# heiheishuang/MuDG

Hardware: AMD Instinct MI355X
Metric: DDIM denoise steps/sec, MDM1024 576x1024x16f (CFG: 2 UNet forwards + fused update per step, per clip) (higher is better)
Workload: dtype bf16; 1 GPU; MDM1024 latents (B=1,4,16,72,128) + c_concat 8ch, context (B,333,1024), 50-step uniform_trailing DDIM schedule, cfg 7.5, guidance_rescale 0.7, eta 1.0, v-prediction, dynamic rescale; clips_per_gpu=1, parallelism=clip-DP x1 (no in-step collective), launch=hipGraph replay of each UNet pass (cond+uncond batched)

## Files before the change

### mudg_amd/csrc/attention.hip

```cpp
#include "attn_shared.h"
#include <cstdlib>

namespace {

#if MUDG_PLANES == 1
template <bool TWO>
__global__ __launch_bounds__(256, 2) void attn_kernel(const MudgAttnDesc p, const int nqt, const int total) {
    __shared__ __attribute__((aligned(16))) h16 Ks[2 * ATILE];
    __shared__ __attribute__((aligned(16))) h16 Vs[2 * ATILE];

    const int tid = threadIdx.x, lane = tid & 63, wave = tid >> 6;
    const int l31 = lane & 31, hi = lane >> 5;

    const int w = xcd_work_item(total);
    const int pair = w / nqt, qt = w - pair * nqt;
    const int f = pair / p.heads, h = pair - f * p.heads;
    const h16* Qp = reinterpret_cast<const h16*>(p.Q) + (int64_t)f * p.Nq * p.ldq + h * 64;
    h16* Op = reinterpret_cast<h16*>(p.O) + (int64_t)f * p.Nq * p.ldo + h * 64;

    const int q = qt * QB + wave * 32 + l31;
    const bool qok = q < p.Nq;

    h16x8 qf[1][4];
    load_q_frags(qf[0], Qp, q, p.ldq, 0, qok, hi);

    const int lrow = tid >> 3, kc = tid & 7;
    u32x4 kr[1][2], vr[1][2];

    f32x16 o[2], res[TWO ? 2 : 1];
    const float c = p.q_prescaled ? 1.0f : p.scale * 1.4426950408889634f;
    float inv = 0.f;
#pragma unroll
    for (int set = 0; set < (TWO ? 2 : 1); ++set) {
        const KvSet kv = kv_set(p, f, h, set);
#pragma unroll
        for (int r = 0; r < 16; ++r) { o[0][r] = 0.f; o[1][r] = 0.f; }
        float m_run = -INFINITY, l_run = 0.f;

        const int nkt = (kv.Nk + KB - 1) / KB;
        load_kv_tile(kv, 0, lrow, kc, kr, vr);
        stage_padded(Ks, Vs, lrow, kc, kr, vr);
        __syncthreads();

        for (int kt = 0; kt < nkt; ++kt) {
            const int cur = kt & 1;
            const bool more = kt + 1 < nkt;
            if (more) load_kv_tile(kv, kt + 1, lrow, kc, kr, vr);
            FLASH_TILE(Ks + cur * ATILE, Vs + cur * ATILE, qf, kt, kv.Nk, c, m_run, l_run, o, l31, hi);
            if (more) stage_padded(Ks + (cur ^ 1) * ATILE, Vs + (cur ^ 1) * ATILE, lrow, kc, kr, vr);
            __syncthreads();
        }
        inv = finish_set<TWO>(p, set, f, h, q, qok, hi, c, m_run, l_run, o, res);
    }
    if (qok) store_o16(o, inv, Op + (int64_t)q * p.ldo, hi, p.accumulate);
}

constexpr int XK_TILES = 3;
template <bool TWO>
__global__ __launch_bounds__(256, 2) void xattn_kernel(const MudgAttnDesc p, const int nqt, const int xq, const int nqc, const int total) {
    extern __shared__ __attribute__((aligned(16))) h16 xlds[];
    h16* Ks = xlds;
    h16* Vs = xlds + XK_TILES * ATILE;
    const int tid = threadIdx.x, lane = tid & 63, wave = tid >> 6;
    const int l31 = lane & 31, hi = lane >> 5;
    const int w = xcd_work_item(total);
    const int pair = w / nqc, qc = w - pair * nqc;
    const int f = pair / p.heads, h = pair - f * p.heads;
    const h16* Qp = reinterpret_cast<const h16*>(p.Q) + (int64_t)f * p.Nq * p.ldq + h * 64;
    h16* Op = reinterpret_cast<h16*>(p.O) + (int64_t)f * p.Nq * p.ldo + h * 64;
    const int nt0 = (p.Nk + KB - 1) / KB;

    {
        const int lrow = tid >> 3, kc = tid & 7;
#pragma unroll
        for (int set = 0; set < (TWO ? 2 : 1); ++set) {
            const KvSet kv = kv_set(p, f, h, set);
            const int nkt = (kv.Nk + KB - 1) / KB;
            for (int kt = 0; kt < nkt; ++kt) {
                const int ti = set == 0 ? kt : nt0 + kt;
                u32x4 kr[1][2], vr[1][2];
                load_kv_tile(kv, kt, lrow, kc, kr, vr);
                stage_padded(Ks + ti * ATILE, Vs + ti * ATILE, lrow, kc, kr, vr);
            }
        }
    }
    __syncthreads();

    const float c = p.q_prescaled ? 1.0f : p.scale * 1.4426950408889634f;
    for (int qi = 0; qi < xq; ++qi) {
        const int qt = qc * xq + qi;
        if (qt >= nqt) break;
        const int q = qt * QB + wave * 32 + l31;
        const bool qok = q < p.Nq;
        h16x8 qf[1][4];
        load_q_frags(qf[0], Qp, q, p.ldq, 0, qok, hi);
        f32x16 o[2], res[TWO ? 2 : 1];
        float inv = 0.f;
#pragma unroll
        for (int set = 0; set < (TWO ? 2 : 1); ++set) {
            const int Nk = set == 0 ? p.Nk : p.Nk2;
#pragma unroll
            for (int r = 0; r < 16; ++r) { o[0][r] = 0.f; o[1][r] = 0.f; }
            float m_run = -INFINITY, l_run = 0.f;
            const int nkt = (Nk + KB - 1) / KB;
            for (int kt = 0; kt < nkt; ++kt) {
                const int ti = set == 0 ? kt : nt0 + kt;
                FLASH_TILE(Ks + ti * ATILE, Vs + ti * ATILE, qf, kt, Nk, c, m_run, l_run, o, l31, hi);
            }
            inv = finish_set<TWO>(p, set, f, h, q, qok, hi, c, m_run, l_run, o, res);
        }
        if (qok) store_o16(o, inv, Op + (int64_t)q * p.ldo, hi, p.accumulate);
    }
}

__global__ __launch_bounds__(256, 2) void attn64q_kernel(const MudgAttnDesc p, const int nqt, const int total) {
    __shared__ __attribute__((aligned(16))) h16 Ks[2 * ATILE];
    __shared__ __attribute__((aligned(16))) h16 Vs[2 * ATILE];

    const int tid = threadIdx.x, lane = tid & 63, wave = tid >> 6;
    const int l31 = lane & 31, hi = lane >> 5;
    const int w = xcd_work_item(total);
    const int pair = w / nqt, qt = w - pair * nqt;
    const int f = pair / p.heads, h = pair - f * p.heads;
    const KvSet kv = kv_set(p, f, h, 0);

    const h16* Qp = reinterpret_cast<const h16*>(p.Q) + (int64_t)f * p.Nq * p.ldq + h * 64;
    h16* Op = reinterpret_cast<h16*>(p.O) + (int64_t)f * p.Nq * p.ldo + h * 64;

    int qrow[2];
    bool qok[2];
    h16x8 qf[2][4];
#pragma unroll
    for (int qb = 0; qb < 2; ++qb) {
        qrow[qb] = qt * 256 + wave * 64 + qb * 32 + l31;
        qok[qb] = qrow[qb] < p.Nq;
        load_q_frags(qf[qb], Qp, qrow[qb], p.ldq, 0, qok[qb], hi);
    }

    const int lrow = tid >> 3, kc = tid & 7;
    u32x4 kr[1][2], vr[1][2];
    const int vlo = (kc >> 1) * 16 + ((kc & 1) ? 4 : 0), vhi = (kc >> 1) * 16 + ((kc & 1) ? 12 : 8);
    auto stage = [&](int buf) {
#pragma unroll
        for (int i = 0; i < 2; ++i) {
            st16(&Ks[buf * ATILE + (lrow + 32 * i) * ALD + kc * 8], kr[0][i]);
// ... 461 lines not shown
        __builtin_amdgcn_wave_barrier();
#pragma unroll
        for (int s = 0; s < 2; ++s) {
            const int r = lr + 8 * s;
            st16(qs + r * 128 + ((lj ^ (r & 7)) << 4), qn[s]);
            st16(ks + r * 128 + ((lj ^ (r & 7)) << 4), kn[s]);
            const int z = tattn_fz(r >> 2);
            u32x2 lo = {vn[s][0], vn[s][1]}, hi = {vn[s][2], vn[s][3]};
            *reinterpret_cast<u32x2*>(vs + r * 128 + (((2 * lj) ^ z) << 3)) = lo;
            *reinterpret_cast<u32x2*>(vs + r * 128 + (((2 * lj + 1) ^ z) << 3)) = hi;
        }
        __builtin_amdgcn_wave_barrier();
        if (it + 1 < TATTN_ITEMS) fetch(w0 + it + 1);

        float ov[16];
        tattn_item_mfma(qs, ks, vs, c, g, T, scale, ov);
        if (c < T) {
            h16* dst = O + (pix + (int64_t)c * HW) * ldo + h * 64 + g * 8;
#pragma unroll
            for (int half = 0; half < 2; ++half) {
                h16x8 t;
#pragma unroll
                for (int e = 0; e < 8; ++e) t[e] = (h16)ov[half * 8 + e];
                st16(dst + half * 32, as_u32x4(t));
            }
        }
    }
}

constexpr int TSA_KT = 64;
constexpr int TSA_ROWS = 128, TSA_COLS = 192;
constexpr int TSA_STAGE = (TSA_ROWS + TSA_COLS) * TSA_KT * 2;
constexpr int TSA_LDS = 2 * TSA_STAGE;
static_assert(TSA_LDS >= 4 * 2 * 3 * 2048, "the dead stages must hold 4 waves x 2 items x 3 tiles (q, k, v) x 2 KB");

__global__ __launch_bounds__(256, 2) void tsattn_fused_kernel(const h16* __restrict__ X, const h16* __restrict__ W, h16* __restrict__ O,
                                                               const int HW, const int heads, const int C, const int64_t ldx,
                                                               const int64_t ldw, const int64_t ldo, const float scale, const int total) {
    extern __shared__ __attribute__((aligned(16))) char tsa_smem[];
    const int tid = threadIdx.x, lane = tid & 63, wave = tid >> 6;
    const int c = lane & 15, g = lane >> 4;
    const int item = xcd_work_item(total);
    const int tile = item / heads, h = item - tile * heads;
    const int tpc = HW >> 3;
    const int b = tile / tpc, px0 = (tile - b * tpc) << 3;
    const int64_t row0 = (int64_t)b * 16 * HW + px0;

    const int lrow = tid >> 3, lch = tid & 7;
    const h16* src[10];
#pragma unroll
    for (int i = 0; i < 4; ++i) {
        const int r = lrow + 32 * i;
        src[i] = X + (row0 + (int64_t)(r & 15) * HW + (r >> 4)) * ldx + lch * 8;
    }
#pragma unroll
    for (int i = 0; i < 6; ++i) src[4 + i] = W + (int64_t)(h * TSA_COLS + lrow + 32 * i) * ldw + lch * 8;
    const int soff = lrow * 128 + ((lch ^ (lrow & 7)) << 4);

    u32x4 nx[10];
    auto fetch = [&](int kt) {
#pragma unroll
        for (int i = 0; i < 10; ++i) nx[i] = ld16(src[i] + kt * TSA_KT);
    };
    auto stage = [&](char* st) {
#pragma unroll
        for (int i = 0; i < 10; ++i) st16(st + soff + 4096 * i, nx[i]);
    };

    f32x4 acc[2][12];
#pragma unroll
    for (int pi = 0; pi < 2; ++pi)
#pragma unroll
        for (int nb = 0; nb < 12; ++nb) acc[pi][nb] = f32x4{0.f, 0.f, 0.f, 0.f};

    const int nk = C / TSA_KT;
    fetch(0);
    stage(tsa_smem);
    __syncthreads();
    for (int kt = 0; kt < nk; ++kt) {
        const char* cur = tsa_smem + (kt & 1) * TSA_STAGE;
        if (kt + 1 < nk) fetch(kt + 1);
#pragma unroll
        for (int s = 0; s < 2; ++s) {
            const int foff = c * 128 + (((g + 4 * s) ^ (c & 7)) << 4);
            const h16x8 xf0 = as_h16x8(ld16(cur + (32 * wave) * 128 + foff));
            const h16x8 xf1 = as_h16x8(ld16(cur + (32 * wave + 16) * 128 + foff));
#pragma unroll
            for (int nb = 0; nb < 12; ++nb) {
                const h16x8 wf = as_h16x8(ld16(cur + (TSA_ROWS + 16 * nb) * 128 + foff));
                acc[0][nb] = MFMA_16x16x32(wf, xf0, acc[0][nb]);
                acc[1][nb] = MFMA_16x16x32(wf, xf1, acc[1][nb]);
            }
        }
        if (kt + 1 < nk) stage(tsa_smem + ((kt + 1) & 1) * TSA_STAGE);
        __syncthreads();
    }

    char* mine = tsa_smem + wave * (2 * 3 * 2048);
#pragma unroll
    for (int pi = 0; pi < 2; ++pi) {
        char* qs = mine + pi * (3 * 2048);
#pragma unroll
        for (int nb = 0; nb < 12; ++nb) {
            Pack8 t;
#pragma unroll
            for (int i = 0; i < 4; ++i) t.h[i] = (h16)acc[pi][nb][i];
            const int u = 4 * (nb & 3) + g;
            const int off = (nb >> 2) == 2 ? c * 128 + ((u ^ tattn_fz(c >> 2)) << 3)
                                           : c * 128 + (((u >> 1) ^ (c & 7)) << 4) + ((u & 1) << 3);
            *reinterpret_cast<u32x2*>(qs + (nb >> 2) * 2048 + off) = t.u;
        }
    }
    __builtin_amdgcn_wave_barrier();
#pragma unroll
    for (int pi = 0; pi < 2; ++pi) {
        const char* qs = mine + pi * (3 * 2048);
        float ov[16];
        tattn_item_mfma(qs, qs + 2048, qs + 4096, c, g, 16, scale, ov);
        h16* dst = O + (row0 + (int64_t)c * HW + (2 * wave + pi)) * ldo + h * 64 + g * 8;
#pragma unroll
        for (int half = 0; half < 2; ++half) {
            h16x8 t;
#pragma unroll
            for (int e = 0; e < 8; ++e) t[e] = (h16)ov[half * 8 + e];
            st16(dst + half * 32, as_u32x4(t));
        }
    }
}
#endif

#if MUDG_PLANES > 1
template <bool TWO>
__global__ __launch_bounds__(256, PLANES == 2 ? 2 : 1) void attn_split_kernel(const MudgAttnDesc p, const int nqt, const int total) {
    extern __shared__ __attribute__((aligned(16))) char smem_raw[];
    h16* Ks = reinterpret_cast<h16*>(smem_raw);
    h16* Vs = Ks + 2 * PLANES * ATILE;

    const int tid = threadIdx.x, lane = tid & 63, wave = tid >> 6;
    const int l31 = lane & 31, hi = lane >> 5;
    const int w = xcd_work_item(total);
    const int pair = w / nqt, qt = w - pair * nqt;
    const int f = pair / p.heads, h = pair - f * p.heads;
    const int psq = p.ldq / PLANES, pso = p.ldo / PLANES;

    const h16* Qp = reinterpret_cast<const h16*>(p.Q) + (int64_t)f * p.Nq * p.ldq + h * 64;
    h16* Op = reinterpret_cast<h16*>(p.O) + (int64_t)f * p.Nq * p.ldo + h * 64;

    const int q = qt * QB + wave * 32 + l31;
    const bool qok = q < p.Nq;
    h16x8 qf[PLANES][4];
#pragma unroll
    for (int pl = 0; pl < PLANES; ++pl) load_q_frags(qf[pl], Qp, q, p.ldq, pl * psq, qok, hi);

    const int lrow = tid >> 3, kc = tid & 7;
    u32x4 kr[PLANES][2], vr[PLANES][2];

    f32x16 o[2], res[TWO ? 2 : 1];
    const float c = p.q_prescaled ? 1.0f : p.scale * 1.4426950408889634f;
#pragma unroll
    for (int set = 0; set < (TWO ? 2 : 1); ++set) {
// ... 426 lines not shown
#endif
        if (dma_ok) {
#if MUDG_PLANES == 2
            if (const int rc = mudg_lds_opt_in<&attn_split_dma_kernel<true>>(SPLIT_DMA_SMEM, "mudg_attention")) return rc;
            if (const int rc = mudg_lds_opt_in<&attn_split_dma_kernel<false>>(SPLIT_DMA_SMEM, "mudg_attention")) return rc;
            if (d.q_prescaled) hipLaunchKernelGGL(attn_split_dma_kernel<true>, dim3((unsigned)total), dim3(256), SPLIT_DMA_SMEM, s, d, nqt, (int)total);
            else hipLaunchKernelGGL(attn_split_dma_kernel<false>, dim3((unsigned)total), dim3(256), SPLIT_DMA_SMEM, s, d, nqt, (int)total);
#endif
        }
        else if (d.K2) hipLaunchKernelGGL(attn_split_kernel<true>, dim3((unsigned)total), dim3(256), smem, s, d, nqt, (int)total);
        else hipLaunchKernelGGL(attn_split_kernel<false>, dim3((unsigned)total), dim3(256), smem, s, d, nqt, (int)total);
    }
#else
    MUDG_REQUIRE(!d.Q8 || wide, "mudg_attention: the MX-fp8 score path serves the long self-attention kernel only (Nq >= 512, Nk >= 256)");
    if (wide) {
        const int nqt2 = (d.Nq + 255) / 256;
        const int64_t total2 = (int64_t)nqt2 * d.F * d.heads;
        static int dma = -1, lean = -1;
        if (dma < 0) dma = mudg_variant("ATTN_DMA", 1);
        if (lean < 0) lean = mudg_variant("ATTN_LEAN", 1);
        const bool dma_ok = dma && d.Nk % 64 == 0 && (int64_t)d.Nk * d.ldk * 2 < (1ll << 31) && (int64_t)64 * d.ldvt * 2 + (int64_t)d.Nk * 2 < (1ll << 31);
        if (d.Q8) {
            MUDG_REQUIRE(dma_ok && d.q_prescaled && d.K8 && d.Qs && d.Ks && !d.accumulate, "mudg_attention: the MX-fp8 score path needs "
                         "q_prescaled, Nk %% 64 == 0 and all four of Q8 / K8 / Qs / Ks");
            MUDG_REQUIRE((d.ldq8 & 15) == 0 && (d.ldk8 & 15) == 0 && aligned16(d.Q8) && aligned16(d.K8) && d.ldq8 >= d.heads * 64 &&
                         d.ldk8 >= d.heads * 64 && d.ldqs >= d.heads * 2 && d.ldks >= d.heads * 2 && (int64_t)d.Nk * d.ldk8 < (1ll << 31),
                         "mudg_attention: fp8 strides");
            hipLaunchKernelGGL((attn64d_kernel<true, true>), dim3((unsigned)total2), dim3(256), 0, s, d, nqt2, (int)total2);
        }
        else if (dma_ok && d.q_prescaled && lean) hipLaunchKernelGGL((attn64d_kernel<true, false>), dim3((unsigned)total2), dim3(256), 0, s, d, nqt2, (int)total2);
        else if (dma_ok) hipLaunchKernelGGL((attn64d_kernel<false, false>), dim3((unsigned)total2), dim3(256), 0, s, d, nqt2, (int)total2);
        else hipLaunchKernelGGL(attn64q_kernel, dim3((unsigned)total2), dim3(256), 0, s, d, nqt2, (int)total2);
    } else {
        static int xv = -1;
        if (xv < 0) xv = mudg_variant("ATTN_X", 1);
        int xq = (int)(total / 1024);
        xq = xq > 8 ? 8 : xq;
        if (xv && xq >= 2 && d.Nk <= 2 * KB && (!d.K2 || d.Nk2 <= KB)) {
            constexpr int smem = 2 * XK_TILES * ATILE * (int)sizeof(h16);
            if (const int rc = mudg_lds_opt_in<&xattn_kernel<false>>(smem, "mudg_attention")) return rc;
            if (const int rc = mudg_lds_opt_in<&xattn_kernel<true>>(smem, "mudg_attention")) return rc;
            const int nqc = (nqt + xq - 1) / xq;
            const int64_t totx = (int64_t)nqc * d.F * d.heads;
            if (d.K2) hipLaunchKernelGGL(xattn_kernel<true>, dim3((unsigned)totx), dim3(256), smem, s, d, nqt, xq, nqc, (int)totx);
            else hipLaunchKernelGGL(xattn_kernel<false>, dim3((unsigned)totx), dim3(256), smem, s, d, nqt, xq, nqc, (int)totx);
        }
        else if (d.K2) hipLaunchKernelGGL(attn_kernel<true>, dim3((unsigned)total), dim3(256), 0, s, d, nqt, (int)total);
        else hipLaunchKernelGGL(attn_kernel<false>, dim3((unsigned)total), dim3(256), 0, s, d, nqt, (int)total);
    }
#endif
    const int rc = mudg_check_launch("mudg_attention");
    const double bh = (double)d.F * d.heads;
    mudg_prof_end(slot, s, 4.0 * bh * d.Nq * (double)(d.Nk + (d.K2 ? d.Nk2 : 0)) * 64.0,
                  bh * (2.0 * d.Nq + 2.0 * d.Nk / d.kv_div + (d.K2 ? 2.0 * d.Nk2 / d.kv_div2 : 0.0)) * 64.0 * 2.0);
    return rc;
}

#if MUDG_PLANES == 1
namespace {
__global__ __launch_bounds__(256) void quantize_mxfp8_kernel(const h16* __restrict__ X, int ldx, int64_t rows, int nblk,
                                                              unsigned char* __restrict__ Y, int ldy, unsigned char* __restrict__ S, int lds) {
    const int64_t i = (int64_t)blockIdx.x * 256 + threadIdx.x;
    if (i >= rows * nblk) return;
    const int64_t r = i / nblk;
    const int b = (int)(i - r * nblk);
    const h16* src = X + r * ldx + b * 32;
    float v[32];
    float amax = 0.f;
#pragma unroll
    for (int q = 0; q < 4; ++q) {
        const h16x8 t = as_h16x8(ld16(src + q * 8));
#pragma unroll
        for (int e = 0; e < 8; ++e) { v[q * 8 + e] = (float)t[e]; amax = fmaxf(amax, fabsf(v[q * 8 + e])); }
    }
    const int E = mx_block_exponent(amax);
    const float inv = __uint_as_float((unsigned)(127 - E) << 23);
    u32x4 lo, hi4;
#pragma unroll
// ... 55 lines not shown
#endif
    if (T <= 16) launch(tattn_split_kernel<16>, 4);
    else launch(tattn_split_kernel<32>, 4);
#else
    if (T <= 16 && use_mfma) launch(tattn_mfma_kernel, 4 * TATTN_ITEMS);
    else if (T <= 16) launch(tattn_kernel<16>, 4 * TATTN_ITEMS);
    else launch(tattn_kernel<32>, 4 * TATTN_ITEMS);
#endif
    const int rc = mudg_check_launch("mudg_temporal_attention");
    mudg_prof_end(slot, s, 4.0 * total * (double)T * T * 64.0, (double)total * T * 64.0 * 2.0 * 4.0);
    return rc;
}

extern "C" int mudg_temporal_self_attention_ok(int T, int HW, int heads, int C, int64_t ldx, int64_t ldw, int64_t ldo) {
#if MUDG_PLANES == 1
    return T == 16 && HW > 0 && HW % 8 == 0 && heads > 0 && C == heads * 64 && ldx % 8 == 0 && ldw % 8 == 0 && ldo % 8 == 0 && ldx >= C &&
           ldw >= C && ldo >= C;
#else
    (void)T; (void)HW; (void)heads; (void)C; (void)ldx; (void)ldw; (void)ldo;
    return 0;
#endif
}

extern "C" int mudg_temporal_self_attention(const void* X, const void* Wh, void* O, int B, int T, int HW, int heads, int C, int64_t ldx,
                                            int64_t ldw, int64_t ldo, float scale, void* stream) {
#if MUDG_PLANES == 1
    MUDG_REQUIRE(X && Wh && O, "mudg_temporal_self_attention: null pointer");
    MUDG_REQUIRE(B > 0, "mudg_temporal_self_attention: empty problem");
    MUDG_REQUIRE(aligned16(X) && aligned16(Wh) && aligned16(O), "mudg_temporal_self_attention: alignment");
    if (!mudg_temporal_self_attention_ok(T, HW, heads, C, ldx, ldw, ldo))
        MUDG_FAIL(MUDG_EUNSUPPORTED, "mudg_temporal_self_attention: T=%d HW=%d heads=%d C=%d outside the fused kernel (T = 16, HW %% 8 == 0, "
                  "C = 64 heads, dense 16-byte rows): project with mudg_gemm and call mudg_temporal_attention", T, HW, heads, C);
    const int64_t total = (int64_t)B * (HW / 8) * heads;
    MUDG_REQUIRE(total < (1ll << 31), "mudg_temporal_self_attention: grid too large");
    const int rc0 = mudg_lds_opt_in<tsattn_fused_kernel>(TSA_LDS, "mudg_temporal_self_attention");
    if (rc0 != MUDG_OK) return rc0;
    hipStream_t s = reinterpret_cast<hipStream_t>(stream);
    const int slot = mudg_prof_begin(MUDG_FAM_GEMM, s);
    hipLaunchKernelGGL(tsattn_fused_kernel, dim3((unsigned)total), dim3(256), TSA_LDS, s, (const h16*)X, (const h16*)Wh, (h16*)O, HW, heads, C,
                       ldx, ldw, ldo, scale, (int)total);
    const int rc = mudg_check_launch("mudg_temporal_self_attention");
    const double M = (double)B * T * HW;
    mudg_prof_end(slot, s, 2.0 * M * 3.0 * C * C + 4.0 * (double)B * HW * heads * T * T * 64.0, (2.0 * M * C + 3.0 * C * C) * 2.0);
    return rc;
#else
    (void)X; (void)Wh; (void)O; (void)B; (void)T; (void)HW; (void)heads; (void)C; (void)ldx; (void)ldw; (void)ldo; (void)scale; (void)stream;
    MUDG_FAIL(MUDG_EUNSUPPORTED, "mudg_temporal_self_attention: the fused kernel belongs to the 16-bit operand builds");
#endif
}
```

### mudg_amd/csrc/attn_shared.h

```cpp
#pragma once
#include "common.h"
#include <type_traits>

constexpr int QB = 128;
constexpr int KB = 64;
constexpr int ALD = 72;
constexpr int ATILE = 64 * ALD;

struct KvSet {
    const h16* Kp;
    const h16* Vp;
    int Nk, ldk, ldvt;
    int psk, psv;
};
__device__ __forceinline__ KvSet kv_set(const MudgAttnDesc& p, int f, int h, int set) {
    KvSet kv;
    if (set == 0) {
        kv.Kp = reinterpret_cast<const h16*>(p.K) + (int64_t)(f / p.kv_div) * p.Nk * p.ldk + h * 64;
        kv.Vp = reinterpret_cast<const h16*>(p.Vt) + (int64_t)(f / p.kv_div) * p.svt + (int64_t)(h * 64) * p.ldvt;
        kv.Nk = p.Nk; kv.ldk = p.ldk; kv.ldvt = p.ldvt;
    } else {
        kv.Kp = reinterpret_cast<const h16*>(p.K2) + (int64_t)(f / p.kv_div2) * p.Nk2 * p.ldk2 + h * 64;
        kv.Vp = reinterpret_cast<const h16*>(p.Vt2) + (int64_t)(f / p.kv_div2) * p.svt2 + (int64_t)(h * 64) * p.ldvt2;
        kv.Nk = p.Nk2; kv.ldk = p.ldk2; kv.ldvt = p.ldvt2;
// ... 11 lines not shown
__device__ __forceinline__ void load_kv_tile(const KvSet& kv, int kt, int lrow, int kc, u32x4 (&kr)[PLANES][2], u32x4 (&vr)[PLANES][2]) {
    const int j0 = kt * KB;
#pragma unroll
    for (int pl = 0; pl < PLANES; ++pl)
#pragma unroll
        for (int i = 0; i < 2; ++i) {
            const int row = lrow + 32 * i;
            const int j = j0 + row;
            kr[pl][i] = (j < kv.Nk) ? ld16(kv.Kp + (int64_t)j * kv.ldk + pl * kv.psk + kc * 8) : zero16();
            const int jc = j0 + kc * 8;
            u32x4 v = zero16();
            if (jc < kv.Nk) {
                v = ld16(kv.Vp + (int64_t)row * kv.ldvt + pl * kv.psv + jc);
                if (jc + 8 > kv.Nk) {
                    h16x8 hv = as_h16x8(v);
#pragma unroll
                    for (int e = 0; e < 8; ++e) if (jc + e >= kv.Nk) hv[e] = (h16)0.f;
                    v = as_u32x4(hv);
                }
            }
            vr[pl][i] = v;
        }
}
__device__ __forceinline__ void stage_padded(h16* Kt, h16* Vt, int lrow, int kc, const u32x4 (&kr)[PLANES][2], const u32x4 (&vr)[PLANES][2]) {
#pragma unroll
    for (int pl = 0; pl < PLANES; ++pl)
#pragma unroll
        for (int i = 0; i < 2; ++i) {
            st16(&Kt[pl * ATILE + (lrow + 32 * i) * ALD + kc * 8], kr[pl][i]);
            st16(&Vt[pl * ATILE + (lrow + 32 * i) * ALD + kc * 8], vr[pl][i]);
        }
}

__device__ __forceinline__ void mask_ragged(f32x16 (&s)[2], int kt, int Nk, int hi) {
    if (kt * KB + KB > Nk) {
#pragma unroll
        for (int sub = 0; sub < 2; ++sub)
#pragma unroll
            for (int r = 0; r < 16; ++r) {
                const int j = kt * KB + sub * 32 + (r & 3) + 8 * (r >> 2) + 4 * hi;
                if (j >= Nk) s[sub][r] = -INFINITY;
            }
    }
}

__device__ __forceinline__ float row_max32(const f32x16 (&s)[2]) {
    float mx = s[0][0];
#pragma unroll
    for (int r = 1; r < 16; ++r) mx = fmaxf(mx, s[0][r]);
#pragma unroll
    for (int r = 0; r < 16; ++r) mx = fmaxf(mx, s[1][r]);
    return fmaxf(mx, __shfl_xor(mx, 32, 64));
}

__device__ __forceinline__ void put_p(h16x8 (&pk)[PLANES][2][2], int sub, int r, float e) {
    h16 piece[PLANES];
    split_operand(e, piece);
#pragma unroll
    for (int pl = 0; pl < PLANES; ++pl) pk[pl][sub][r >> 3][r & 7] = piece[pl];
}

__device__ __forceinline__ void softmax_step_classic(const f32x16 (&s)[2], float c, float& m_run, float& l_run, f32x16 (&o)[2],
                                                     h16x8 (&pk)[PLANES][2][2]) {
    const float mx = row_max32(s);
    const bool grew = !__all(mx <= m_run);
    const float m_new = grew ? fmaxf(m_run, mx) : m_run;
    const float alpha = grew ? __builtin_amdgcn_exp2f((m_run - m_new) * c) : 1.0f;
    const float mc = m_new * c;
    m_run = m_new;
    float ps = 0.f;
#pragma unroll
    for (int sub = 0; sub < 2; ++sub)
#pragma unroll
        for (int r = 0; r < 16; ++r) {
            const float e = __builtin_amdgcn_exp2f(fmaf(s[sub][r], c, -mc));
            ps += e;
            put_p(pk, sub, r, e);
        }
    l_run = l_run * alpha + ps;
    if (grew) {
#pragma unroll
        for (int r = 0; r < 16; ++r) { o[0][r] *= alpha; o[1][r] *= alpha; }
    }
}

#ifdef MUDG_OPERAND_FP16
constexpr float LEAN_LIMIT = 32768.f;
#else
constexpr float LEAN_LIMIT = 1099511627776.f;
#endif
__device__ __forceinline__ bool softmax_step_lean(const f32x16 (&s)[2], float& l_run, h16x8 (&pk)[PLANES][2][2]) {
    float ps = 0.f;
#pragma unroll
    for (int sub = 0; sub < 2; ++sub)
#pragma unroll
        for (int r = 0; r < 16; ++r) {
            const float e = __builtin_amdgcn_exp2f(s[sub][r]);
            ps += e;
            put_p(pk, sub, r, e);
        }
    l_run += ps;
    return !(ps <= LEAN_LIMIT);
}
template <bool LEAN, class KeyLoop>
__device__ __forceinline__ void lean_or_classic(const bool& overflow, KeyLoop key_loop) {
    if constexpr (LEAN) {
        key_loop(std::true_type{});
        if (__syncthreads_or(overflow ? 1 : 0)) key_loop(std::false_type{});
    } else {
        key_loop(std::false_type{});
    }
}

#define FLASH_TILE(Kt, Vt, qf, kt, Nk, c, m_run, l_run, o, l31, hi) do {                                                  \
    const h16* const ft_K = (Kt); const h16* const ft_V = (Vt); const int ft_kt = (kt), ft_Nk = (Nk);                     \
    f32x16 ft_s[2];                                                                                                       \
    _Pragma("unroll") for (int sub = 0; sub < 2; ++sub) {                                                                 \
        _Pragma("unroll") for (int r = 0; r < 16; ++r) ft_s[sub][r] = 0.f;                                                \
        _Pragma("unroll") for (int sg = 0; sg < NSEG; ++sg) {                                                             \
            const h16* kp = ft_K + seg_xp(sg) * ATILE + (sub * 32 + (l31)) * ALD + (hi) * 8;                              \
            _Pragma("unroll") for (int ks = 0; ks < 4; ++ks) {                                                            \
                const h16x8 kf = *reinterpret_cast<const h16x8*>(kp + ks * 16);                                           \
                ft_s[sub] = MFMA_32x32x16(kf, (qf)[seg_wp(sg)][ks], ft_s[sub]);                                           \
            }                                                                                                             \
        }                                                                                                                 \
    }                                                                                                                     \
    mask_ragged(ft_s, ft_kt, ft_Nk, (hi));                                                                                \
    h16x8 ft_pk[PLANES][2][2];                                                                                            \
    softmax_step_classic(ft_s, (c), (m_run), (l_run), (o), ft_pk);                                                        \
    _Pragma("unroll") for (int dt = 0; dt < 2; ++dt)                                                                      \
        _Pragma("unroll") for (int sg = 0; sg < NSEG; ++sg) {                                                             \
            const h16* vp = ft_V + seg_xp(sg) * ATILE + (dt * 32 + (l31)) * ALD + 4 * (hi);                               \
            _Pragma("unroll") for (int sub = 0; sub < 2; ++sub)                                                           \
                _Pragma("unroll") for (int jj = 0; jj < 2; ++jj) {                                                        \
                    const int kk = sub * 32 + jj * 16;                                                                    \
                    const h16x4 lo = *reinterpret_cast<const h16x4*>(vp + kk);                                            \
                    const h16x4 up = *reinterpret_cast<const h16x4*>(vp + kk + 8);                                        \
                    h16x8 vf;                                                                                             \
                    _Pragma("unroll") for (int e = 0; e < 4; ++e) { vf[e] = lo[e]; vf[4 + e] = up[e]; }                   \
                    (o)[dt] = MFMA_32x32x16(vf, ft_pk[seg_wp(sg)][sub][jj], (o)[dt]);                                     \
                }                                                                                                         \
        }                                                                                                                 \
} while (0)

__device__ __forceinline__ void store_lse(const MudgAttnDesc& p, int f, int h, int q, bool qok, int hi, float c, float m_run, float l_tot) {
    if (p.Lse && qok && hi == 0) p.Lse[((int64_t)f * p.Nq + q) * p.heads + h] = m_run * c + __log2f(l_tot);
}
__device__ __forceinline__ void store_o16(const f32x16 (&o)[2], float inv, h16* orow, int hi, int accumulate) {
#pragma unroll
    for (int dt = 0; dt < 2; ++dt)
#pragma unroll
        for (int g = 0; g < 4; ++g) {
            h16* dst = orow + dt * 32 + 8 * g + 4 * hi;
            float v[4];
#pragma unroll
            for (int j = 0; j < 4; ++j) v[j] = o[dt][4 * g + j] * inv;
            if (accumulate) {
                Pack8 old; old.u = *reinterpret_cast<const u32x2*>(dst);
#pragma unroll
                for (int j = 0; j < 4; ++j) v[j] += (float)old.h[j];
            }
            Pack8 nw;
#pragma unroll
            for (int j = 0; j < 4; ++j) nw.h[j] = (h16)v[j];
            *reinterpret_cast<u32x2*>(dst) = nw.u;
        }
}
template <bool TWO>
__device__ __forceinline__ float finish_set(const MudgAttnDesc& p, int set, int f, int h, int q, bool qok, int hi, float c,
                                            float m_run, float l_run, f32x16 (&o)[2], f32x16 (&res)[TWO ? 2 : 1]) {
    const float l_tot = l_run + __shfl_xor(l_run, 32, 64);
    float inv = 1.f / l_tot;
    if (!TWO) store_lse(p, f, h, q, qok, hi, c, m_run, l_tot);
    if (TWO) {
        if (set == 0) {
#pragma unroll
            for (int r = 0; r < 16; ++r) { res[0][r] = o[0][r] * inv; res[1][r] = o[1][r] * inv; }
        } else {
#pragma unroll
            for (int r = 0; r < 16; ++r) { o[0][r] = fmaf(o[0][r], inv, res[0][r]); o[1][r] = fmaf(o[1][r], inv, res[1][r]); }
            inv = 1.f;
        }
    }
    return inv;
}
__device__ __forceinline__ void finish_block16(const MudgAttnDesc& p, int f, int h, int q, bool qok, int hi, float c,
                                               float m_run, float l_run, const f32x16 (&o)[2], h16* Op) {
    const float l_tot = l_run + __shfl_xor(l_run, 32, 64);
    const float inv = 1.f / l_tot;
    store_lse(p, f, h, q, qok, hi, c, m_run, l_tot);
    if (qok) store_o16(o, inv, Op + (int64_t)q * p.ldo, hi, p.accumulate);
}

__device__ __forceinline__ __amdgpu_buffer_rsrc_t attn_rsrc(const h16* base) {
    return __builtin_amdgcn_make_buffer_rsrc(const_cast<h16*>(base), 0, (int)0x80000000u, 0x00020000);
}
typedef __attribute__((address_space(3))) void* attn_lptr_t;
__device__ __forceinline__ int swap_mid4(int row) {
    const int i16 = row & 15;
    return (row & ~15) | (i16 & 3) | ((i16 & 8) >> 1) | ((i16 & 4) << 1);
// ... 11 lines not shown
```

Baseline: 8.790 steps/s.

## Make fused temporal self-attention persistent with async LDS buffer loads

Converts the fused temporal self-attention kernel from one workgroup per item into a persistent grid of two workgroups per CU, each walking a contiguous range of items. Operand tiles are now fetched with buffer loads that write straight to LDS, interleaved with the MFMA loop, and the next item's first stage is prefetched while the current item's attention epilogue runs. This is meant to remove register staging, launch tail effects and the exposed load latency at item boundaries. It adds hand-placed vmcnt waits and barriers with fixed counts, and an out-of-bounds offset trick for the final prefetch, which are fragile if the tile shape changes.

```diff
diff --git a/mudg_amd/csrc/attention.hip b/mudg_amd/csrc/attention.hip
--- a/mudg_amd/csrc/attention.hip
+++ b/mudg_amd/csrc/attention.hip
@@ -638,100 +638,145 @@
 constexpr int TSA_ROWS = 128, TSA_COLS = 192;
 constexpr int TSA_STAGE = (TSA_ROWS + TSA_COLS) * TSA_KT * 2;
 constexpr int TSA_LDS = 2 * TSA_STAGE;
-static_assert(TSA_LDS >= 4 * 2 * 3 * 2048, "the dead stages must hold 4 waves x 2 items x 3 tiles (q, k, v) x 2 KB");
+constexpr int TSA_XP = TSA_ROWS / 8 / 4, TSA_WP = TSA_COLS / 8 / 4;
+constexpr int TSA_STORES = 2 * 2;
+constexpr unsigned TSA_OOB = 0x80000000u;
+static_assert(TSA_STAGE >= 4 * 3 * 2048, "a dead stage must hold 4 waves x 3 tiles (q, k, v) x 2 KB");
+static_assert(TSA_XP + TSA_WP == 10 && TSA_STORES == 4, "TSA_WAIT_ITEM below is TSA_STORES");
+#define TSA_WAIT_STAGE() asm volatile("s_waitcnt vmcnt(0)" ::: "memory")
+#define TSA_WAIT_ITEM() asm volatile("s_waitcnt vmcnt(4)" ::: "memory")
+#define TSA_BARRIER()                          \
+    do {                                       \
+        __builtin_amdgcn_sched_barrier(0);     \
+        __builtin_amdgcn_s_barrier();          \
+        __builtin_amdgcn_sched_barrier(0);     \
+    } while (0)
 
 __global__ __launch_bounds__(256, 2) void tsattn_fused_kernel(const h16* __restrict__ X, const h16* __restrict__ W, h16* __restrict__ O,
                                                                const int HW, const int heads, const int C, const int64_t ldx,
                                                                const int64_t ldw, const int64_t ldo, const float scale, const int total) {
     extern __shared__ __attribute__((aligned(16))) char tsa_smem[];
-    const int tid = threadIdx.x, lane = tid & 63, wave = tid >> 6;
+    const int tid = threadIdx.x, lane = tid & 63;
+    const int wave = __builtin_amdgcn_readfirstlane(tid >> 6);
     const int c = lane & 15, g = lane >> 4;
-    const int item = xcd_work_item(total);
-    const int tile = item / heads, h = item - tile * heads;
-    const int tpc = HW >> 3;
-    const int b = tile / tpc, px0 = (tile - b * tpc) << 3;
-    const int64_t row0 = (int64_t)b * 16 * HW + px0;
-
-    const int lrow = tid >> 3, lch = tid & 7;
-    const h16* src[10];
-#pragma unroll
-    for (int i = 0; i < 4; ++i) {
-        const int r = lrow + 32 * i;
-        src[i] = X + (row0 + (int64_t)(r & 15) * HW + (r >> 4)) * ldx + lch * 8;
-    }
-#pragma unroll
-    for (int i = 0; i < 6; ++i) src[4 + i] = W + (int64_t)(h * TSA_COLS + lrow + 32 * i) * ldw + lch * 8;
-    const int soff = lrow * 128 + ((lch ^ (lrow & 7)) << 4);
-
-    u32x4 nx[10];
-    auto fetch = [&](int kt) {
-#pragma unroll
-        for (int i = 0; i < 10; ++i) nx[i] = ld16(src[i] + kt * TSA_KT);
-    };
-    auto stage = [&](char* st) {
-#pragma unroll
-        for (int i = 0; i < 10; ++i) st16(st + soff + 4096 * i, nx[i]);
+    const int nwg = (int)gridDim.x, wg = xcd_work_item(nwg);
+    const int per = total / nwg, rem = total % nwg;
+    const int i0 = wg * per + (wg < rem ? wg : rem), i1 = i0 + per + (wg < rem ? 1 : 0);
+    if (i0 == i1) return;
+    const int nk = C / TSA_KT;
+
+    auto next_item = [&](int& h, int& px0, int& b) {
+        if (++h == heads) {
+            h = 0;
+            px0 += 8;
+            if (px0 == HW) { px0 = 0; ++b; }
+        }
+    };
+    int h, px0, b;
+    {
+        const int tile = i0 / heads, tpc = HW >> 3;
+        h = i0 - tile * heads;
+        b = tile / tpc;
+        px0 = (tile - b * tpc) << 3;
+    }
+    int nit = i0, nkt = 0, nh = h, npx0 = px0, nb = b;
+
+    const int lrow = lane >> 3, lch = (lane & 7) ^ lrow;
+    const int ldx2 = (int)ldx * 2, ldw2 = (int)ldw * 2;
+    const unsigned vx = (unsigned)lrow * (unsigned)HW * (unsigned)ldx2 + (unsigned)lch * 16u;
+    const unsigned vw = (unsigned)lrow * (unsigned)ldw2 + (unsigned)lch * 16u;
+    __amdgpu_buffer_rsrc_t rX, rW;
+    unsigned ux, uw;
+    int ko;
+    auto aim = [&]() {
+        const bool live = nit < i1;
+        rX = attn_rsrc(X + ((int64_t)nb * 16 * HW + npx0) * ldx);
+        rW = attn_rsrc(W + (int64_t)nh * TSA_COLS * ldw);
+        ux = live ? vx : TSA_OOB, uw = live ? vw : TSA_OOB;
+        ko = nkt * (TSA_KT * 2);
+    };
+    auto piece = [&](char* buf, const int j) {
+        if (j < TSA_XP)
+            __builtin_amdgcn_raw_ptr_buffer_load_lds(rX, (attn_lptr_t)(buf + (TSA_XP * wave + j) * 1024), 16, (int)ux,
+                                                     ((j & 1) * 8 * HW + 2 * wave + (j >> 1)) * ldx2 + ko, 0, 0);
+        else
+            __builtin_amdgcn_raw_ptr_buffer_load_lds(rW, (attn_lptr_t)(buf + (TSA_ROWS / 8 + TSA_WP * wave + (j - TSA_XP)) * 1024), 16, (int)uw,
+                                                     (8 * TSA_WP * wave + 8 * (j - TSA_XP)) * ldw2 + ko, 0, 0);
+    };
+    auto advance = [&]() {
+        if (++nkt == nk) { nkt = 0; ++nit; next_item(nh, npx0, nb); }
+    };
+    auto issue = [&](char* buf) {
+        aim();
+#pragma unroll
+        for (int j = 0; j < TSA_XP + TSA_WP; ++j) piece(buf, j);
+        advance();
     };
 
     f32x4 acc[2][12];
 #pragma unroll
     for (int pi = 0; pi < 2; ++pi)
 #pragma unroll
-        for (int nb = 0; nb < 12; ++nb) acc[pi][nb] = f32x4{0.f, 0.f, 0.f, 0.f};
-
-    const int nk = C / TSA_KT;
-    fetch(0);
-    stage(tsa_smem);
-    __syncthreads();
-    for (int kt = 0; kt < nk; ++kt) {
-        const char* cur = tsa_smem + (kt & 1) * TSA_STAGE;
-        if (kt + 1 < nk) fetch(kt + 1);
-#pragma unroll
-        for (int s = 0; s < 2; ++s) {
-            const int foff = c * 128 + (((g + 4 * s) ^ (c & 7)) << 4);
-            const h16x8 xf0 = as_h16x8(ld16(cur + (32 * wave) * 128 + foff));
-            const h16x8 xf1 = as_h16x8(ld16(cur + (32 * wave + 16) * 128 + foff));
-#pragma unroll
-            for (int nb = 0; nb < 12; ++nb) {
-                const h16x8 wf = as_h16x8(ld16(cur + (TSA_ROWS + 16 * nb) * 128 + foff));
-                acc[0][nb] = MFMA_16x16x32(wf, xf0, acc[0][nb]);
-                acc[1][nb] = MFMA_16x16x32(wf, xf1, acc[1][nb]);
-            }
-        }
-        if (kt + 1 < nk) stage(tsa_smem + ((kt + 1) & 1) * TSA_STAGE);
-        __syncthreads();
-    }
-
-    char* mine = tsa_smem + wave * (2 * 3 * 2048);
-#pragma unroll
-    for (int pi = 0; pi < 2; ++pi) {
-        char* qs = mine + pi * (3 * 2048);
-#pragma unroll
-        for (int nb = 0; nb < 12; ++nb) {
-            Pack8 t;
-#pragma unroll
-            for (int i = 0; i < 4; ++i) t.h[i] = (h16)acc[pi][nb][i];
-            const int u = 4 * (nb & 3) + g;
-            const int off = (nb >> 2) == 2 ? c * 128 + ((u ^ tattn_fz(c >> 2)) << 3)
-                                           : c * 128 + (((u >> 1) ^ (c & 7)) << 4) + ((u & 1) << 3);
-            *reinterpret_cast<u32x2*>(qs + (nb >> 2) * 2048 + off) = t.u;
-        }
-    }
-    __builtin_amdgcn_wave_barrier();
-#pragma unroll
-    for (int pi = 0; pi < 2; ++pi) {
-        const char* qs = mine + pi * (3 * 2048);
-        float ov[16];
-        tattn_item_mfma(qs, qs + 2048, qs + 4096, c, g, 16, scale, ov);
-        h16* dst = O + (row0 + (int64_t)c * HW + (2 * wave + pi)) * ldo + h * 64 + g * 8;
-#pragma unroll
-        for (int half = 0; half < 2; ++half) {
-            h16x8 t;
-#pragma unroll
-            for (int e = 0; e < 8; ++e) t[e] = (h16)ov[half * 8 + e];
-            st16(dst + half * 32, as_u32x4(t));
-        }
-    }
+        for (int nb_ = 0; nb_ < 12; ++nb_) acc[pi][nb_] = f32x4{0.f, 0.f, 0.f, 0.f};
+
+    int par = 0;
+    issue(tsa_smem);
+    for (int it = i0; it < i1; ++it) {
+        for (int kt = 0; kt < nk; ++kt) {
+            if (kt == 0 && it != i0) TSA_WAIT_ITEM(); else TSA_WAIT_STAGE();
+            TSA_BARRIER();
+            const char* cur = tsa_smem + par * TSA_STAGE;
+            par ^= 1;
+            char* nxt = tsa_smem + par * TSA_STAGE;
+            aim();
+#pragma unroll
+            for (int s = 0; s < 2; ++s) {
+                const int foff = c * 128 + (((g + 4 * s) ^ (c & 7)) << 4);
+                const h16x8 xf0 = as_h16x8(ld16(cur + (32 * wave) * 128 + foff));
+                const h16x8 xf1 = as_h16x8(ld16(cur + (32 * wave + 16) * 128 + foff));
+#pragma unroll
+                for (int nb_ = 0; nb_ < 12; ++nb_) {
+                    const h16x8 wf = as_h16x8(ld16(cur + (TSA_ROWS + 16 * nb_) * 128 + foff));
+                    acc[0][nb_] = MFMA_16x16x32(wf, xf0, acc[0][nb_]);
+                    acc[1][nb_] = MFMA_16x16x32(wf, xf1, acc[1][nb_]);
+                    if ((nb_ & 1) == 1 && 6 * s + (nb_ >> 1) < TSA_XP + TSA_WP) piece(nxt, 6 * s + (nb_ >> 1));
+                }
+            }
+            advance();
+            __builtin_amdgcn_sched_barrier(0);
+        }
+
+        TSA_BARRIER();
+        char* qs = tsa_smem + (par ^ 1) * TSA_STAGE + wave * (3 * 2048);
+        h16* dst = O + ((int64_t)b * 16 * HW + px0 + (int64_t)c * HW + 2 * wave) * ldo + h * 64 + g * 8;
+#pragma unroll
+        for (int pi = 0; pi < 2; ++pi) {
+            __builtin_amdgcn_wave_barrier();
+#pragma unroll
+            for (int nb_ = 0; nb_ < 12; ++nb_) {
+                Pack8 t;
+#pragma unroll
+                for (int i = 0; i < 4; ++i) t.h[i] = (h16)acc[pi][nb_][i];
+                acc[pi][nb_] = f32x4{0.f, 0.f, 0.f, 0.f};
+                const int u = 4 * (nb_ & 3) + g;
+                const int off = (nb_ >> 2) == 2 ? c * 128 + ((u ^ tattn_fz(c >> 2)) << 3)
+                                                : c * 128 + (((u >> 1) ^ (c & 7)) << 4) + ((u & 1) << 3);
+                *reinterpret_cast<u32x2*>(qs + (nb_ >> 2) * 2048 + off) = t.u;
+            }
+            __builtin_amdgcn_wave_barrier();
+            float ov[16];
+            tattn_item_mfma(qs, qs + 2048, qs + 4096, c, g, 16, scale, ov);
+#pragma unroll
+            for (int half = 0; half < 2; ++half) {
+                h16x8 t;
+#pragma unroll
+                for (int e = 0; e < 8; ++e) t[e] = (h16)ov[half * 8 + e];
+                st16(dst + pi * ldo + half * 32, as_u32x4(t));
+            }
+        }
+        next_item(h, px0, b);
+    }
+    TSA_WAIT_STAGE();
 }
 #endif
 
@@ -1357,12 +1402,16 @@
         MUDG_FAIL(MUDG_EUNSUPPORTED, "mudg_temporal_self_attention: T=%d HW=%d heads=%d C=%d outside the fused kernel (T = 16, HW %% 8 == 0, "
                   "C = 64 heads, dense 16-byte rows): project with mudg_gemm and call mudg_temporal_attention", T, HW, heads, C);
     const int64_t total = (int64_t)B * (HW / 8) * heads;
-    MUDG_REQUIRE(total < (1ll << 31), "mudg_temporal_self_attention: grid too large");
+    MUDG_REQUIRE(total < (1ll << 31), "mudg_temporal_self_attention: too many items");
+    MUDG_REQUIRE(16 * (int64_t)HW * ldx * 2 < (1ll << 31) && (int64_t)TSA_COLS * ldw * 2 < (1ll << 31),
+                 "mudg_temporal_self_attention: a tile spans 2 GiB or more");
     const int rc0 = mudg_lds_opt_in<tsattn_fused_kernel>(TSA_LDS, "mudg_temporal_self_attention");
     if (rc0 != MUDG_OK) return rc0;
+    const int cus = mudg_cu_count();
+    const int grid = 2 * ((cus < 8 ? 256 : cus) & ~7);
     hipStream_t s = reinterpret_cast<hipStream_t>(stream);
     const int slot = mudg_prof_begin(MUDG_FAM_GEMM, s);
-    hipLaunchKernelGGL(tsattn_fused_kernel, dim3((unsigned)total), dim3(256), TSA_LDS, s, (const h16*)X, (const h16*)Wh, (h16*)O, HW, heads, C,
+    hipLaunchKernelGGL(tsattn_fused_kernel, dim3((unsigned)grid), dim3(256), TSA_LDS, s, (const h16*)X, (const h16*)Wh, (h16*)O, HW, heads, C,
                        ldx, ldw, ldo, scale, (int)total);
     const int rc = mudg_check_launch("mudg_temporal_self_attention");
     const double M = (double)B * T * HW;
```

After: 8.821 steps/s, median of 6. About the same (+0.4%).

## Prefetch next Q tile, half-tile ragged tail, and wide O stores in cross-attention

Applied to the files above, without the earlier changes.

In the cross-attention kernel that keeps K/V resident in LDS, the Q fragments for the next query tile are now loaded while the current tile computes, which hides global load latency. When the last key tile is at most half full, it runs through a single-sub FLASH_TILE variant so the fully masked half is skipped. Outputs are packed with permlane32_swap into 16-byte stores when not accumulating. It also lets ATTN_X override the query chunk size. The cost is extra registers for the prefetched Q, which may lower occupancy.

```diff
diff --git a/mudg_amd/csrc/attention.hip b/mudg_amd/csrc/attention.hip
--- a/mudg_amd/csrc/attention.hip
+++ b/mudg_amd/csrc/attention.hip
@@ -56,7 +56,7 @@
 }
 
 constexpr int XK_TILES = 3;
-template <bool TWO>
+template <bool TWO, bool PIPE>
 __global__ __launch_bounds__(256, 2) void xattn_kernel(const MudgAttnDesc p, const int nqt, const int xq, const int nqc, const int total) {
     extern __shared__ __attribute__((aligned(16))) h16 xlds[];
     h16* Ks = xlds;
@@ -69,6 +69,11 @@
     const h16* Qp = reinterpret_cast<const h16*>(p.Q) + (int64_t)f * p.Nq * p.ldq + h * 64;
     h16* Op = reinterpret_cast<h16*>(p.O) + (int64_t)f * p.Nq * p.ldo + h * 64;
     const int nt0 = (p.Nk + KB - 1) / KB;
+    const int qt0 = qc * xq, qt1 = qt0 + xq < nqt ? qt0 + xq : nqt;
+    const int qlane = wave * 32 + l31;
+
+    h16x8 qnext[4];
+    if constexpr (PIPE) load_q_frags(qnext, Qp, qt0 * QB + qlane, p.ldq, 0, qt0 * QB + qlane < p.Nq, hi);
 
     {
         const int lrow = tid >> 3, kc = tid & 7;
@@ -87,13 +92,19 @@
     __syncthreads();
 
     const float c = p.q_prescaled ? 1.0f : p.scale * 1.4426950408889634f;
-    for (int qi = 0; qi < xq; ++qi) {
-        const int qt = qc * xq + qi;
-        if (qt >= nqt) break;
-        const int q = qt * QB + wave * 32 + l31;
+    const bool wide_o = PIPE && !p.accumulate && (p.ldo & 7) == 0;
+    for (int qt = qt0; qt < qt1; ++qt) {
+        const int q = qt * QB + qlane;
         const bool qok = q < p.Nq;
         h16x8 qf[1][4];
-        load_q_frags(qf[0], Qp, q, p.ldq, 0, qok, hi);
+        if constexpr (PIPE) {
+#pragma unroll
+            for (int ks = 0; ks < 4; ++ks) qf[0][ks] = qnext[ks];
+            const int qn = q + QB;
+            load_q_frags(qnext, Qp, qn, p.ldq, 0, qt + 1 < qt1 && qn < p.Nq, hi);
+        } else {
+            load_q_frags(qf[0], Qp, q, p.ldq, 0, qok, hi);
+        }
         f32x16 o[2], res[TWO ? 2 : 1];
         float inv = 0.f;
 #pragma unroll
@@ -103,14 +114,30 @@
             for (int r = 0; r < 16; ++r) { o[0][r] = 0.f; o[1][r] = 0.f; }
             float m_run = -INFINITY, l_run = 0.f;
             const int nkt = (Nk + KB - 1) / KB;
-            for (int kt = 0; kt < nkt; ++kt) {
+            const int nfull = PIPE && (nkt - 1) * KB + KB / 2 >= Nk ? nkt - 1 : nkt;
+            for (int kt = 0; kt < nfull; ++kt) {
                 const int ti = set == 0 ? kt : nt0 + kt;
                 FLASH_TILE(Ks + ti * ATILE, Vs + ti * ATILE, qf, kt, Nk, c, m_run, l_run, o, l31, hi);
             }
+            if (nfull < nkt) {
+                const int ti = set == 0 ? nfull : nt0 + nfull;
+                FLASH_TILE_SUBS(1, Ks + ti * ATILE, Vs + ti * ATILE, qf, nfull, Nk, c, m_run, l_run, o, l31, hi);
+            }
             inv = finish_set<TWO>(p, set, f, h, q, qok, hi, c, m_run, l_run, o, res);
         }
-        if (qok) store_o16(o, inv, Op + (int64_t)q * p.ldo, hi, p.accumulate);
-    }
+        if (wide_o) store_o16_wide(o, inv, Op + (int64_t)q * p.ldo, hi, qok);
+        else if (qok) store_o16(o, inv, Op + (int64_t)q * p.ldo, hi, p.accumulate);
+    }
+}
+
+template <bool TWO, bool PIPE>
+int xattn_launch(const MudgAttnDesc& d, int nqt, int xq, hipStream_t s) {
+    constexpr int smem = 2 * XK_TILES * ATILE * (int)sizeof(h16);
+    if (const int rc = mudg_lds_opt_in<&xattn_kernel<TWO, PIPE>>(smem, "mudg_attention")) return rc;
+    const int nqc = (nqt + xq - 1) / xq;
+    const int64_t totx = (int64_t)nqc * d.F * d.heads;
+    hipLaunchKernelGGL((xattn_kernel<TWO, PIPE>), dim3((unsigned)totx), dim3(256), smem, s, d, nqt, xq, nqc, (int)totx);
+    return MUDG_OK;
 }
 
 __global__ __launch_bounds__(256, 2) void attn64q_kernel(const MudgAttnDesc p, const int nqt, const int total) {
@@ -1224,18 +1251,17 @@
         else if (dma_ok) hipLaunchKernelGGL((attn64d_kernel<false, false>), dim3((unsigned)total2), dim3(256), 0, s, d, nqt2, (int)total2);
         else hipLaunchKernelGGL(attn64q_kernel, dim3((unsigned)total2), dim3(256), 0, s, d, nqt2, (int)total2);
     } else {
-        static int xv = -1;
+        static int xv = -1, xpipe = -1;
         if (xv < 0) xv = mudg_variant("ATTN_X", 1);
+        if (xpipe < 0) xpipe = mudg_variant("ATTN_XPIPE", 1);
         int xq = (int)(total / 1024);
         xq = xq > 8 ? 8 : xq;
+        if (xv >= 2) xq = xv;
         if (xv && xq >= 2 && d.Nk <= 2 * KB && (!d.K2 || d.Nk2 <= KB)) {
-            constexpr int smem = 2 * XK_TILES * ATILE * (int)sizeof(h16);
-            if (const int rc = mudg_lds_opt_in<&xattn_kernel<false>>(smem, "mudg_attention")) return rc;
-            if (const int rc = mudg_lds_opt_in<&xattn_kernel<true>>(smem, "mudg_attention")) return rc;
-            const int nqc = (nqt + xq - 1) / xq;
-            const int64_t totx = (int64_t)nqc * d.F * d.heads;
-            if (d.K2) hipLaunchKernelGGL(xattn_kernel<true>, dim3((unsigned)totx), dim3(256), smem, s, d, nqt, xq, nqc, (int)totx);
-            else hipLaunchKernelGGL(xattn_kernel<false>, dim3((unsigned)totx), dim3(256), smem, s, d, nqt, xq, nqc, (int)totx);
+            int rc;
+            if (xpipe) rc = d.K2 ? xattn_launch<true, true>(d, nqt, xq, s) : xattn_launch<false, true>(d, nqt, xq, s);
+            else rc = d.K2 ? xattn_launch<true, false>(d, nqt, xq, s) : xattn_launch<false, false>(d, nqt, xq, s);
+            if (rc) return rc;
         }
         else if (d.K2) hipLaunchKernelGGL(attn_kernel<true>, dim3((unsigned)total), dim3(256), 0, s, d, nqt, (int)total);
         else hipLaunchKernelGGL(attn_kernel<false>, dim3((unsigned)total), dim3(256), 0, s, d, nqt, (int)total);
diff --git a/mudg_amd/csrc/attn_shared.h b/mudg_amd/csrc/attn_shared.h
--- a/mudg_amd/csrc/attn_shared.h
+++ b/mudg_amd/csrc/attn_shared.h
@@ -67,10 +67,11 @@
         }
 }
 
-__device__ __forceinline__ void mask_ragged(f32x16 (&s)[2], int kt, int Nk, int hi) {
+template <int NS>
+__device__ __forceinline__ void mask_ragged(f32x16 (&s)[NS], int kt, int Nk, int hi) {
     if (kt * KB + KB > Nk) {
 #pragma unroll
-        for (int sub = 0; sub < 2; ++sub)
+        for (int sub = 0; sub < NS; ++sub)
 #pragma unroll
             for (int r = 0; r < 16; ++r) {
                 const int j = kt * KB + sub * 32 + (r & 3) + 8 * (r >> 2) + 4 * hi;
@@ -79,12 +80,15 @@
     }
 }
 
-__device__ __forceinline__ float row_max32(const f32x16 (&s)[2]) {
+template <int NS>
+__device__ __forceinline__ float row_max32(const f32x16 (&s)[NS]) {
     float mx = s[0][0];
 #pragma unroll
     for (int r = 1; r < 16; ++r) mx = fmaxf(mx, s[0][r]);
 #pragma unroll
-    for (int r = 0; r < 16; ++r) mx = fmaxf(mx, s[1][r]);
+    for (int sub = 1; sub < NS; ++sub)
+#pragma unroll
+        for (int r = 0; r < 16; ++r) mx = fmaxf(mx, s[sub][r]);
     return fmaxf(mx, __shfl_xor(mx, 32, 64));
 }
 
@@ -95,7 +99,8 @@
     for (int pl = 0; pl < PLANES; ++pl) pk[pl][sub][r >> 3][r & 7] = piece[pl];
 }
 
-__device__ __forceinline__ void softmax_step_classic(const f32x16 (&s)[2], float c, float& m_run, float& l_run, f32x16 (&o)[2],
+template <int NS>
+__device__ __forceinline__ void softmax_step_classic(const f32x16 (&s)[NS], float c, float& m_run, float& l_run, f32x16 (&o)[2],
                                                      h16x8 (&pk)[PLANES][2][2]) {
     const float mx = row_max32(s);
     const bool grew = !__all(mx <= m_run);
@@ -105,7 +110,7 @@
     m_run = m_new;
     float ps = 0.f;
 #pragma unroll
-    for (int sub = 0; sub < 2; ++sub)
+    for (int sub = 0; sub < NS; ++sub)
 #pragma unroll
         for (int r = 0; r < 16; ++r) {
             const float e = __builtin_amdgcn_exp2f(fmaf(s[sub][r], c, -mc));
@@ -147,10 +152,11 @@
     }
 }
 
-#define FLASH_TILE(Kt, Vt, qf, kt, Nk, c, m_run, l_run, o, l31, hi) do {                                                  \
+#define FLASH_TILE(Kt, Vt, qf, kt, Nk, c, m_run, l_run, o, l31, hi) FLASH_TILE_SUBS(2, Kt, Vt, qf, kt, Nk, c, m_run, l_run, o, l31, hi)
+#define FLASH_TILE_SUBS(NS, Kt, Vt, qf, kt, Nk, c, m_run, l_run, o, l31, hi) do {                                         \
     const h16* const ft_K = (Kt); const h16* const ft_V = (Vt); const int ft_kt = (kt), ft_Nk = (Nk);                     \
-    f32x16 ft_s[2];                                                                                                       \
-    _Pragma("unroll") for (int sub = 0; sub < 2; ++sub) {                                                                 \
+    f32x16 ft_s[NS];                                                                                                      \
+    _Pragma("unroll") for (int sub = 0; sub < (NS); ++sub) {                                                              \
         _Pragma("unroll") for (int r = 0; r < 16; ++r) ft_s[sub][r] = 0.f;                                                \
         _Pragma("unroll") for (int sg = 0; sg < NSEG; ++sg) {                                                             \
             const h16* kp = ft_K + seg_xp(sg) * ATILE + (sub * 32 + (l31)) * ALD + (hi) * 8;                              \
@@ -166,7 +172,7 @@
     _Pragma("unroll") for (int dt = 0; dt < 2; ++dt)                                                                      \
         _Pragma("unroll") for (int sg = 0; sg < NSEG; ++sg) {                                                             \
             const h16* vp = ft_V + seg_xp(sg) * ATILE + (dt * 32 + (l31)) * ALD + 4 * (hi);                               \
-            _Pragma("unroll") for (int sub = 0; sub < 2; ++sub)                                                           \
+            _Pragma("unroll") for (int sub = 0; sub < (NS); ++sub)                                                        \
                 _Pragma("unroll") for (int jj = 0; jj < 2; ++jj) {                                                        \
                     const int kk = sub * 32 + jj * 16;                                                                    \
                     const h16x4 lo = *reinterpret_cast<const h16x4*>(vp + kk);                                            \
@@ -201,6 +207,29 @@
             *reinterpret_cast<u32x2*>(dst) = nw.u;
         }
 }
+__device__ __forceinline__ void store_o16_wide(const f32x16 (&o)[2], float inv, h16* orow, int hi, bool qok) {
+#pragma unroll
+    for (int dt = 0; dt < 2; ++dt)
+#pragma unroll
+        for (int g = 0; g < 4; g += 2) {
+            Pack8 nw[2];
+#pragma unroll
+            for (int b = 0; b < 2; ++b)
+#pragma unroll
+                for (int j = 0; j < 4; ++j) {
+                    float v = o[dt][4 * (g + b) + j] * inv;
+                    asm volatile("" : "+v"(v));
+                    nw[b].h[j] = (h16)v;
+                }
+            u32x4 bits;
+#pragma unroll
+            for (int d = 0; d < 2; ++d) {
+                const auto sw = __builtin_amdgcn_permlane32_swap(nw[0].u[d], nw[1].u[d], false, false);
+                bits[d] = sw[0]; bits[2 + d] = sw[1];
+            }
+            if (qok) st16(orow + dt * 32 + 8 * (g + hi), bits);
+        }
+}
 template <bool TWO>
 __device__ __forceinline__ float finish_set(const MudgAttnDesc& p, int set, int f, int h, int q, bool qok, int hi, float c,
                                             float m_run, float l_run, f32x16 (&o)[2], f32x16 (&res)[TWO ? 2 : 1]) {
```

Measured after the change: 8.252 steps/s before, 8.270 steps/s after, median of 6. No clear change (+0.2%).
